# ydchen0806/CLC

Measured on AMD Instinct MI355X. Metric: images/sec fwd+bwd @256x256 bs8; bpp+PSNR parity vs ref, higher is better.
Workload: dtype f32; 1 GPU; CLC N=64 lambda=0.0067 MSE, 256x256 bs8/GPU, n_refs=1: fwd + RD loss + bwd + clip_grad_norm + AdamW + aux step (configs[1]); global_batch=8, parallelism=dp1, ranks_seen=1, collective=none, hip_graph=True

## Files before the change

clc_amd/csrc/conv_wino.hip:

```cpp
#include "common.h"

namespace {
#include "conv_common.h"

constexpr int TH = 8, TW = 16, HW = TW + 2, HPIX = (TH + 2) * HW;
constexpr int HALO_FLOATS = HPIX * 128;
constexpr int PIECES = HPIX / 2;

struct WinoParams {
  ConvParams c;
  const float* u;
  int items, ntn, ncg;
  unsigned u_bytes;
};

#ifndef WINO_AB
#define WINO_AB 0
#endif
#if WINO_AB & 32
__device__ unsigned long long wino_dbg[32];
#define WINO_STAMP(k) do { if (blockIdx.x == 0 && tid == 0 && it == i0 + 1) wino_dbg[k] = __builtin_amdgcn_s_memtime(); } while (0)
#else
#define WINO_STAMP(k) do { } while (0)
#endif
#define MFMA(a, b, c) __builtin_amdgcn_mfma_f32_32x32x2f32((a), (b), (c), 0, 0, 0)

constexpr int VB_FLOATS = 16 * 32 * 16;

template <bool SHUF>
__global__ __launch_bounds__(512, 1) void conv_wino_kernel(const WinoParams wp) {
  const ConvParams& p = wp.c;
  extern __shared__ __attribute__((aligned(16))) float smem[];
  float* halo = smem;
  float* bias_s = smem + HALO_FLOATS + 2 * VB_FLOATS;
  float* VV = smem + HALO_FLOATS;
  const int tid = threadIdx.x, lane = tid & 63, wave = tid >> 6;
  const int li = lane & 31, h = lane >> 5;
  const int tiles_w = p.W / TW, tiles_h = p.H / TH;
  const int KCT = wp.ncg * 4;
  const int NC16 = wp.ncg * 8;
  const int i0 = (int)((long)wp.items * blockIdx.x / gridDim.x), i1 = (int)((long)wp.items * (blockIdx.x + 1) / gridDim.x);
  const __amdgpu_buffer_rsrc_t xr = __builtin_amdgcn_make_buffer_rsrc(const_cast<float*>(p.x), 0, p.x_bytes, 0x00020000);
  const __amdgpu_buffer_rsrc_t ur = __builtin_amdgcn_make_buffer_rsrc(const_cast<float*>(wp.u), 0, wp.u_bytes, 0x00020000);
  const int q = tid & 3, t = (tid >> 2) & 31, part = tid >> 7;
  const int ty = t >> 3, tx = t & 7;
  const int wi = wave >> 1, nh = wave & 1;
  const int qo = tid & 15, to = tid >> 4;
  const int ra = part == 0 ? 0 : (part == 2 ? 2 : 1), rb = part == 0 ? 2 : (part == 1 ? 2 : (part == 2 ? 1 : 3));
  const float sg = part == 1 ? 1.f : -1.f;
  const int hbase = ((2 * ty + ra) * HW + 2 * tx) * 128, hdelta = (rb - ra) * HW * 128;
  const int sw0 = (tx & 3) << 2, sw1 = ((tx + 1) & 3) << 2;
  const int vdst = (part * 4 * 32 + t) * 16 + ((q ^ ((t >> 2) & 3)) << 2);
  int afo[2];
#pragma unroll
  for (int t8 = 0; t8 < 2; ++t8) afo[t8] = li * 16 + (((2 * t8 + h) ^ ((li >> 2) & 3)) << 2);
  const unsigned b_lane = (unsigned)lane * 16u;
  const bool lean = epilogue_is_lean(p);

  auto deposit = [&](int pt, int cg) {
    const int txx = pt % tiles_w, t2 = pt / tiles_w, tyy = t2 % tiles_h, n = t2 / tiles_h;
    const int oy0 = tyy * TH, ox0 = txx * TW;
    const int org = ((n * p.H + oy0 - 1) * p.W + ox0 - 1) * p.ldx + cg * 128;
    int hy = 0, hx = 2 * wave + h;
#pragma unroll 1
    for (int pc = wave; pc < PIECES; pc += 8) {
      const int iy = oy0 - 1 + hy, ix = ox0 - 1 + hx;
      const bool ok = (unsigned)iy < (unsigned)p.H && (unsigned)ix < (unsigned)p.W;
      const int c = li ^ (((hx >> 1) & 3) << 2);
      dma16(xr, halo + pc * 256, ok ? (unsigned)(org + (hy * p.W + hx) * p.ldx + c * 4) * 4u : kOOB);
      hx += 16;
      if (hx >= HW) { hx -= HW; ++hy; }
    }
  };

  int res_pt = -1, res_cg = -1;
  for (int it = i0; it < i1; ++it) {
    const int pt = it / wp.ntn, nt = it - pt * wp.ntn;
    const int txx = pt % tiles_w, t2 = pt / tiles_w, tyy = t2 % tiles_h, n = t2 / tiles_h;
    const int oy0 = tyy * TH, ox0 = txx * TW;
    f32x16 acc[4][2];
#pragma unroll
    for (int jj = 0; jj < 4; ++jj)
#pragma unroll
      for (int nbi = 0; nbi < 2; ++nbi)
#pragma unroll
        for (int r = 0; r < 16; ++r) acc[jj][nbi][r] = 0.f;
    f32x4 bq[2][2][2];
    auto load_b = [&](int slot, int jj, int c16) {
      const int kcg = c16 >> 1, t8g = 2 * (c16 & 1);
#pragma unroll
      for (int nbi = 0; nbi < 2; ++nbi) {
        const unsigned base = (unsigned)(((((nt * 16 + 4 * wi + jj) * KCT + kcg) * 4 + 2 * nh + nbi) * 4 + t8g)) * 1024u;
#pragma unroll
        for (int t8 = 0; t8 < 2; ++t8) bq[slot][nbi][t8] = buf_load4(ur, b_lane + base + (unsigned)(t8 * 1024));
      }
    };
    const float bias_v = (p.bias && tid < 128) ? p.bias[nt * 128 + tid] : 0.f;
    load_b(0, 0, 0);
    WINO_STAMP(0);

    for (int cg = 0; cg < wp.ncg; ++cg) {
      bool landed = cg == 0;
      if (pt != res_pt || cg != res_cg) {
        res_pt = pt; res_cg = cg;
        deposit(pt, cg);
        landed = false;
      }
      if (!landed) asm volatile("s_waitcnt vmcnt(0)" ::: "memory");
      __syncthreads();
      WINO_STAMP(1);
      if (cg == 0 && tid < 128) bias_s[tid] = bias_v;
      {
        f32x4 T[4];
#pragma unroll
        for (int c = 0; c < 4; ++c) {
          const float* src = halo + hbase + c * 128 + ((q ^ (c < 2 ? sw0 : sw1)) << 2);
          T[c] = *reinterpret_cast<const f32x4*>(src) + sg * *reinterpret_cast<const f32x4*>(src + hdelta);
        }
        float* dst = VV + vdst;
        *reinterpret_cast<f32x4*>(dst) = T[0] - T[2];
        *reinterpret_cast<f32x4*>(dst + 1 * 32 * 16) = T[1] + T[2];
        *reinterpret_cast<f32x4*>(dst + 2 * 32 * 16) = T[2] - T[1];
        *reinterpret_cast<f32x4*>(dst + 3 * 32 * 16) = T[1] - T[3];
      }
      WINO_STAMP(2);
#pragma unroll 1
      for (int kc = 0; kc < 8; ++kc) {
        __syncthreads();
        WINO_STAMP(3 + kc);
        const float* Vc = VV + (kc & 1) * VB_FLOATS;
        float* Vn = VV + ((kc + 1) & 1) * VB_FLOATS;
        const int c16 = cg * 8 + kc;
        f32x4 aq[2][2];
        f32x4 da[4], T[4];
#pragma unroll
        for (int t8 = 0; t8 < 2; ++t8) aq[0][t8] = *reinterpret_cast<const f32x4*>(Vc + (4 * wi) * 512 + afo[t8]);
        int npt = -1, ncg2 = 0;
        if (kc == 7) {
          npt = pt; ncg2 = cg + 1;
          if (ncg2 == wp.ncg) { ncg2 = 0; npt = it + 1 < i1 ? (it + 1) / wp.ntn : -1; }
          if (npt >= 0 && (npt != res_pt || ncg2 != res_cg)) { res_pt = npt; res_cg = ncg2; } else npt = -1;
          if (npt >= 0) deposit(npt, ncg2);
        }
#pragma unroll
        for (int g = 0; g < 4; ++g) {
          const int cur = g & 1;
          if (!(WINO_AB & 4)) {
            if (g < 3) load_b(cur ^ 1, g + 1, c16);
            else load_b(cur ^ 1, 0, c16 + 1 < NC16 ? c16 + 1 : 0);
          }
          if (g < 3) {
#pragma unroll
            for (int t8 = 0; t8 < 2; ++t8) aq[cur ^ 1][t8] = *reinterpret_cast<const f32x4*>(Vc + (4 * wi + g + 1) * 512 + afo[t8]);
          }
          if (WINO_AB & 8) {
          } else if (g == 0) {
            const int cb = (((kc + 1) & 7) * 4 + q);
#pragma unroll
            for (int c = 0; c < 4; ++c) da[c] = *reinterpret_cast<const f32x4*>(halo + hbase + c * 128 + ((cb ^ (c < 2 ? sw0 : sw1)) << 2));
          } else if (g == 1) {
            const int cb = (((kc + 1) & 7) * 4 + q);
#pragma unroll
            for (int c = 0; c < 4; ++c) {
              const f32x4 dbv = *reinterpret_cast<const f32x4*>(halo + hbase + hdelta + c * 128 + ((cb ^ (c < 2 ? sw0 : sw1)) << 2));
              T[c] = da[c] + sg * dbv;
            }
          } else if (g == 2) {
            float* dst = Vn + vdst;
            *reinterpret_cast<f32x4*>(dst) = T[0] - T[2];
            *reinterpret_cast<f32x4*>(dst + 1 * 32 * 16) = T[1] + T[2];
            *reinterpret_cast<f32x4*>(dst + 2 * 32 * 16) = T[2] - T[1];
            *reinterpret_cast<f32x4*>(dst + 3 * 32 * 16) = T[1] - T[3];
          }
          __builtin_amdgcn_sched_barrier(0);
#pragma unroll
          for (int t8 = 0; t8 < 2; ++t8)
#pragma unroll
            for (int ss = 0; ss < 4; ++ss)
#pragma unroll
              for (int nbi = 0; nbi < 2; ++nbi) {
                if (!(WINO_AB & 1)) acc[g][nbi] = MFMA(aq[cur][t8][ss], bq[cur][nbi][t8][ss], acc[g][nbi]);
                else acc[g][nbi][(t8 * 4 + ss) & 15] += aq[cur][t8][ss] * bq[cur][nbi][t8][ss];
              }
          __builtin_amdgcn_sched_barrier(0);
        }
      }
    }
    WINO_STAMP(11);
    asm volatile("s_waitcnt vmcnt(0)" ::: "memory");
    WINO_STAMP(12);
#pragma unroll 1
    for (int rd = 0; rd < ((WINO_AB & 2) ? 1 : 2); ++rd) {
      const int tyo = to >> 3, txo = to & 7;
      const int co = nt * 128 + ((qo >> 3) * 2 + rd) * 32 + (qo & 7) * 4;
      const f32x4 bv = *reinterpret_cast<const f32x4*>(bias_s + (co - nt * 128));
      __syncthreads();
      WINO_STAMP(13 + 3 * rd);
#pragma unroll
      for (int b = 0; b < 2; ++b) {
        float* dst = VV + ((wi * 2 + b) * 32) * 64;
#pragma unroll
        for (int r = 0; r < 16; ++r) {
          const float m0 = rd == 0 ? acc[0][0][r] : acc[0][1][r], m1 = rd == 0 ? acc[1][0][r] : acc[1][1][r];
          const float m2 = rd == 0 ? acc[2][0][r] : acc[2][1][r], m3 = rd == 0 ? acc[3][0][r] : acc[3][1][r];
          const float cv = b == 0 ? (m0 + m1) + m2 : (m1 - m2) - m3;
          const int row = (r & 3) + 8 * (r >> 2) + 4 * h;
          dst[row * 64 + ((nh * 32 + li) ^ (h << 5))] = cv;
        }
      }
      __syncthreads();
      WINO_STAMP(14 + 3 * rd);
      {
        const int col = (qo << 2) ^ (((to >> 2) & 1) << 5);
        f32x4 y[2][2];
#pragma unroll
        for (int b = 0; b < 2; ++b) {
          f32x4 c[4];
#pragma unroll
          for (int ii = 0; ii < 4; ++ii) c[ii] = *reinterpret_cast<const f32x4*>(VV + ((ii * 2 + b) * 32 + to) * 64 + col);
          y[0][b] = (c[0] + c[1]) + c[2];
          y[1][b] = (c[1] - c[2]) - c[3];
        }
        const int mrow0 = (n * p.OH + oy0 + 2 * tyo) * p.OW + ox0 + 2 * txo;
        if (lean) {
          if (!SHUF) {
#pragma unroll 1
            for (int a = 0; a < 2; ++a) {
              const size_t pix = (size_t)(mrow0 + a * p.OW);
              const f32x4 ya = a ? y[1][0] : y[0][0], yb = a ? y[1][1] : y[0][1];
              const Lean4In ia = lean_load4(p, pix, co), ib = lean_load4(p, pix + 1, co);
              lean_finish4(p, bv, ya, ia, pix, co);
              lean_finish4(p, bv, yb, ib, pix + 1, co);
            }
          } else {
#pragma unroll 1
            for (int a = 0; a < 2; ++a) {
              const f32x4 ya = a ? y[1][0] : y[0][0], yb = a ? y[1][1] : y[0][1];
              lean_store_shuffle4(p, bv, ya, n, oy0 + 2 * tyo + a, ox0 + 2 * txo, co);
              lean_store_shuffle4(p, bv, yb, n, oy0 + 2 * tyo + a, ox0 + 2 * txo + 1, co);
            }
          }
        } else if (!SHUF) {
#pragma unroll 1
          for (int a = 0; a < 2; ++a) {
            const size_t pix = (size_t)(mrow0 + a * p.OW);
            const f32x4 ya = a ? y[1][0] : y[0][0], yb = a ? y[1][1] : y[0][1];
            const Epi4In ia = epilogue_load4(p, pix, co), ib = epilogue_load4(p, pix + 1, co);
            epilogue_finish4(p, bv, ya, ia, pix, co);
            epilogue_finish4(p, bv, yb, ib, pix + 1, co);
          }
        } else {
#pragma unroll 1
          for (int a = 0; a < 2; ++a)
#pragma unroll 1
            for (int e = 0; e < 4; ++e) {
              epilogue_store(p, a ? y[1][0][e] : y[0][0][e], bv[e], mrow0 + a * p.OW, co + e, p.OH, p.OW, 0, 0);
              epilogue_store(p, a ? y[1][1][e] : y[0][1][e], bv[e], mrow0 + a * p.OW + 1, co + e, p.OH, p.OW, 0, 0);
            }
        }
      }
      WINO_STAMP(15 + 3 * rd);
    }
  }
}

constexpr int HALO2_FLOATS = HPIX * 64;
constexpr int V2_FLOATS = 16 * 32 * 16;
constexpr int PIECES2 = HPIX / 4;

template <bool SHUF>
__global__ __launch_bounds__(256, 2) void conv_wino64_kernel(const WinoParams wp) {
  const ConvParams& p = wp.c;
  extern __shared__ __attribute__((aligned(16))) float smem[];
  float* halo = smem;
  float* V = smem + HALO2_FLOATS;
  float* S = smem;
  const int tid = threadIdx.x, lane = tid & 63, wave = tid >> 6;
  const int li = lane & 31, h = lane >> 5;
  const int tiles_w = p.W / TW, tiles_h = p.H / TH;
  const int KCT = wp.ncg * 2;
  const int NC16 = wp.ncg * 4;
  const int i0 = (int)((long)wp.items * blockIdx.x / gridDim.x), i1 = (int)((long)wp.items * (blockIdx.x + 1) / gridDim.x);
  const __amdgpu_buffer_rsrc_t xr = __builtin_amdgcn_make_buffer_rsrc(const_cast<float*>(p.x), 0, p.x_bytes, 0x00020000);
  const __amdgpu_buffer_rsrc_t ur = __builtin_amdgcn_make_buffer_rsrc(const_cast<float*>(wp.u), 0, wp.u_bytes, 0x00020000);
  const int q = tid & 3, t = (tid >> 2) & 31, half = tid >> 7;
  const int ty = t >> 3, tx = t & 7;
  const int qo = tid & 15;
  const bool lean = epilogue_is_lean(p);
  int afo[2];
#pragma unroll
  for (int t8 = 0; t8 < 2; ++t8) afo[t8] = li * 16 + (((2 * t8 + h) ^ ((li >> 2) & 3)) << 2);
  const unsigned b_lane = (unsigned)lane * 16u;

  int cur_pt = -1, cur_cg = -1;
  for (int it = i0; it < i1; ++it) {
    const int pt = it / wp.ntn, nt = it - pt * wp.ntn;
    const int txx = pt % tiles_w, t2 = pt / tiles_w, tyy = t2 % tiles_h, n = t2 / tiles_h;
    const int oy0 = tyy * TH, ox0 = txx * TW;
    f32x16 acc[4][2];
#pragma unroll
    for (int s = 0; s < 4; ++s)
#pragma unroll
      for (int nb = 0; nb < 2; ++nb)
#pragma unroll
        for (int r = 0; r < 16; ++r) acc[s][nb][r] = 0.f;
    f32x4 bq[2][2][2];
    auto load_b = [&](int slot, int s, int c16) {
      const int kcg = c16 >> 1, t8g = 2 * (c16 & 1);
#pragma unroll
      for (int nb = 0; nb < 2; ++nb) {
        const unsigned base = (unsigned)((((((nt >> 1) * 16 + 4 * wave + s) * KCT + kcg) * 4 + 2 * (nt & 1) + nb) * 4 + t8g)) * 1024u;
#pragma unroll
        for (int t8 = 0; t8 < 2; ++t8) bq[slot][nb][t8] = buf_load4(ur, b_lane + base + (unsigned)(t8 * 1024));
      }
    };
    load_b(0, 0, 0);

    for (int cg = 0; cg < wp.ncg; ++cg) {
      if (pt != cur_pt || cg != cur_cg) {
        cur_pt = pt; cur_cg = cg;
        const int org = ((n * p.H + oy0 - 1) * p.W + ox0 - 1) * p.ldx + cg * 64;
        int hy = 0, hx = 4 * wave + (lane >> 4);
#pragma unroll 1
        for (int pc = wave; pc < PIECES2; pc += 4) {
          const int iy = oy0 - 1 + hy, ix = ox0 - 1 + hx;
          const bool ok = (unsigned)iy < (unsigned)p.H && (unsigned)ix < (unsigned)p.W;
          const int c = (lane & 15) ^ (((hx >> 1) & 3) << 2);
          dma16(xr, halo + pc * 256, ok ? (unsigned)(org + (hy * p.W + hx) * p.ldx + c * 4) * 4u : kOOB);
          hx += 16;
          if (hx >= HW) { hx -= HW; ++hy; }
        }
        asm volatile("s_waitcnt vmcnt(0)" ::: "memory");
      }
#pragma unroll 1
      for (int kc = 0; kc < 4; ++kc) {
        __syncthreads();
        {
          const int cidx = kc * 4 + q;
          f32x4 d[3][4];
#pragma unroll
          for (int r = 0; r < 3; ++r)
#pragma unroll
            for (int c = 0; c < 4; ++c) {
              const int hy = 2 * ty + r + half, hx = 2 * tx + c;
              d[r][c] = *reinterpret_cast<const f32x4*>(halo + (hy * HW + hx) * 64 + ((cidx ^ (((hx >> 1) & 3) << 2)) << 2));
            }
          f32x4 T[2][4];
#pragma unroll
          for (int c = 0; c < 4; ++c) {
            if (half == 0) { T[0][c] = d[0][c] - d[2][c]; T[1][c] = d[1][c] + d[2][c]; }
            else           { T[0][c] = d[1][c] - d[0][c]; T[1][c] = d[0][c] - d[2][c]; }
          }
#pragma unroll
          for (int i = 0; i < 2; ++i) {
            const f32x4 v0 = T[i][0] - T[i][2], v1 = T[i][1] + T[i][2], v2 = T[i][2] - T[i][1], v3 = T[i][1] - T[i][3];
            float* dst = V + (((2 * half + i) * 4) * 32 + t) * 16 + ((q ^ ((t >> 2) & 3)) << 2);
            *reinterpret_cast<f32x4*>(dst) = v0;
            *reinterpret_cast<f32x4*>(dst + 1 * 32 * 16) = v1;
            *reinterpret_cast<f32x4*>(dst + 2 * 32 * 16) = v2;
            *reinterpret_cast<f32x4*>(dst + 3 * 32 * 16) = v3;
          }
        }
        __syncthreads();
        const int c16 = cg * 4 + kc;
        f32x4 aq[2][2];
#pragma unroll
        for (int t8 = 0; t8 < 2; ++t8) aq[0][t8] = *reinterpret_cast<const f32x4*>(V + (4 * wave) * 512 + afo[t8]);
#pragma unroll
        for (int s = 0; s < 4; ++s) {
          const int cur = s & 1;
          if (s < 3) {
            load_b(cur ^ 1, s + 1, c16);
#pragma unroll
            for (int t8 = 0; t8 < 2; ++t8) aq[cur ^ 1][t8] = *reinterpret_cast<const f32x4*>(V + (4 * wave + s + 1) * 512 + afo[t8]);
          } else {
            load_b(cur ^ 1, 0, c16 + 1 < NC16 ? c16 + 1 : 0);
          }
          __builtin_amdgcn_sched_barrier(0);
#pragma unroll
          for (int t8 = 0; t8 < 2; ++t8)
#pragma unroll
            for (int ss = 0; ss < 4; ++ss)
#pragma unroll
              for (int nb = 0; nb < 2; ++nb) acc[s][nb] = MFMA(aq[cur][t8][ss], bq[cur][nb][t8][ss], acc[s][nb]);
          __builtin_amdgcn_sched_barrier(0);
        }
      }
    }
    cur_pt = -1;
    {
      const int co = nt * 64 + (qo >> 3) * 32 + (qo & 7) * 4;
      const f32x4 bv = epilogue_bias4(p.bias, co);
      __syncthreads();
#pragma unroll
      for (int b = 0; b < 2; ++b) {
        float* dst = S + ((wave * 2 + b) * 32) * 64;
#pragma unroll
        for (int nb = 0; nb < 2; ++nb)
#pragma unroll
          for (int r = 0; r < 16; ++r) {
            const float cv = b == 0 ? (acc[0][nb][r] + acc[1][nb][r]) + acc[2][nb][r] : (acc[1][nb][r] - acc[2][nb][r]) - acc[3][nb][r];
            const int row = (r & 3) + 8 * (r >> 2) + 4 * h;
            dst[row * 64 + ((nb * 32 + li) ^ (h << 5))] = cv;
          }
      }
      __syncthreads();
#pragma unroll 1
      for (int tt = 0; tt < 2; ++tt) {
        const int to = (tid >> 4) + 16 * tt, tyo = to >> 3, txo = to & 7;
        const int col = (qo << 2) ^ (((to >> 2) & 1) << 5);
        f32x4 y[2][2];
#pragma unroll
        for (int b = 0; b < 2; ++b) {
          f32x4 c[4];
#pragma unroll
          for (int ii = 0; ii < 4; ++ii) c[ii] = *reinterpret_cast<const f32x4*>(S + ((ii * 2 + b) * 32 + to) * 64 + col);
          y[0][b] = (c[0] + c[1]) + c[2];
          y[1][b] = (c[1] - c[2]) - c[3];
        }
        const int mrow0 = (n * p.OH + oy0 + 2 * tyo) * p.OW + ox0 + 2 * txo;
#pragma unroll 1
        for (int a = 0; a < 2; ++a) {
          const size_t pix = (size_t)(mrow0 + a * p.OW);
          const f32x4 ya = a ? y[1][0] : y[0][0], yb = a ? y[1][1] : y[0][1];
          if (lean) {
            if (!SHUF) {
              const Lean4In ia = lean_load4(p, pix, co), ib = lean_load4(p, pix + 1, co);
              lean_finish4(p, bv, ya, ia, pix, co);
              lean_finish4(p, bv, yb, ib, pix + 1, co);
            } else {
              lean_store_shuffle4(p, bv, ya, n, oy0 + 2 * tyo + a, ox0 + 2 * txo, co);
              lean_store_shuffle4(p, bv, yb, n, oy0 + 2 * tyo + a, ox0 + 2 * txo + 1, co);
            }
          } else if (!SHUF) {
            const Epi4In ia = epilogue_load4(p, pix, co), ib = epilogue_load4(p, pix + 1, co);
            epilogue_finish4(p, bv, ya, ia, pix, co);
            epilogue_finish4(p, bv, yb, ib, pix + 1, co);
          } else {
#pragma unroll 1
            for (int e = 0; e < 4; ++e) {
              epilogue_store(p, ya[e], bv[e], (int)pix, co + e, p.OH, p.OW, 0, 0);
              epilogue_store(p, yb[e], bv[e], (int)pix + 1, co + e, p.OH, p.OW, 0, 0);
            }
          }
        }
      }
    }
    __syncthreads();
  }
}

__device__ __forceinline__ void wino_u_one(const float* __restrict__ w, float* __restrict__ out, long e, int K, int flip) {
  const int kq = (int)(e % (K / 4)), n = (int)(e / (K / 4)), k = kq * 4;
  f32x4 g[3][3];
#pragma unroll
  for (int a = 0; a < 3; ++a)
#pragma unroll
    for (int b = 0; b < 3; ++b) {
      const int tap = flip ? 8 - (a * 3 + b) : a * 3 + b;
      g[a][b] = *reinterpret_cast<const f32x4*>(w + ((size_t)n * 9 + tap) * K + k);
    }
  f32x4 tt[4][3];
#pragma unroll
  for (int b = 0; b < 3; ++b) {
    tt[0][b] = g[0][b];
    tt[1][b] = 0.5f * ((g[0][b] + g[1][b]) + g[2][b]);
    tt[2][b] = 0.5f * ((g[0][b] - g[1][b]) + g[2][b]);
    tt[3][b] = g[2][b];
  }
  const int KCT = K / 32, nt = n >> 7, nb = (n & 127) >> 5, kcg = k >> 5, kk = k & 31, t8 = kk >> 3, hh = (kk & 7) >> 2;
  const int lane = (n & 31) + 32 * hh;
#pragma unroll
  for (int i = 0; i < 4; ++i) {
    f32x4 u[4];
    u[0] = tt[i][0];
    u[1] = 0.5f * ((tt[i][0] + tt[i][1]) + tt[i][2]);
    u[2] = 0.5f * ((tt[i][0] - tt[i][1]) + tt[i][2]);
    u[3] = tt[i][2];
#pragma unroll
    for (int j = 0; j < 4; ++j) {
      const size_t idx = ((((((size_t)nt * 16 + (i * 4 + j)) * KCT + kcg) * 4 + nb) * 4 + t8) * 64 + lane);
      *reinterpret_cast<f32x4*>(out + idx * 4) = u[j];
    }
  }
}
__global__ void filter_wino_kernel(const float* __restrict__ w, float* __restrict__ out, int N, int K, int flip) {
  const long e = (long)blockIdx.x * blockDim.x + threadIdx.x;
  if (e >= (long)N * K / 4) return;
  wino_u_one(w, out, e, K, flip);
}
__global__ void filter_wino_batched_kernel(const clc_wino_entry* __restrict__ table, int n_entries) {
  int lo = 0, hi = n_entries - 1;
  const int b = blockIdx.x;
  while (lo < hi) {
    const int mid = (lo + hi + 1) >> 1;
    if (table[mid].block_begin <= b) lo = mid; else hi = mid - 1;
  }
  const clc_wino_entry en = table[lo];
  const long e = (long)(b - en.block_begin) * blockDim.x + threadIdx.x;
  if (e >= (long)en.N * en.K / 4) return;
  wino_u_one(en.w, en.out, e, en.K, en.flip);
}

}

extern "C" int clc_filter_wino(const float* w, float* out, int N, int K, int flip, clc_stream_t stream) {
  CLC_CHECK(w && out && N > 0 && N % 64 == 0 && K > 0 && K % 64 == 0 && aligned16(w) && aligned16(out),
            "clc_filter_wino: rows and channels must be positive multiples of 64, pointers 16-B aligned (got N=%d K=%d)", N, K);
  const long total = (long)N * K / 4;
  hipLaunchKernelGGL(filter_wino_kernel, dim3((unsigned)((total + 255) / 256)), dim3(256), 0, (hipStream_t)stream, w, out, N, K, flip);
  CLC_LAUNCH_CHECK();
  return 0;
}
extern "C" int clc_filter_wino_batched(const clc_wino_entry* table_dev, int n_entries, int total_blocks, clc_stream_t stream) {
  CLC_CHECK(table_dev && n_entries > 0 && total_blocks > 0, "clc_filter_wino_batched: bad args");
  hipLaunchKernelGGL(filter_wino_batched_kernel, dim3(total_blocks), dim3(256), 0, (hipStream_t)stream, table_dev, n_entries);
  CLC_LAUNCH_CHECK();
  return 0;
}

int clc_conv_wino_launch(const void* conv_params, const float* u, hipStream_t st) {
  const ConvParams& p = *reinterpret_cast<const ConvParams*>(conv_params);
  if (!u || p.ks != 3 || p.stride != 1 || p.pad != 1 || p.Cin % 64 || p.Cin > 1024 || p.Cout % 64 || p.H % TH || p.W % TW || p.OH != p.H || p.OW != p.W) return 0;
  if (p.xs || p.in_op != CLC_IN_NONE || p.group_rows || p.bf16 || p.ksplit > 1 || p.ldx % 4 || !aligned16(p.x) || !aligned16(u)) return 0;
  const bool shuf = p.shuffle != 0;
  if (!shuf && !p.vec_epi) return 0;
  const size_t ub = (size_t)((p.Cout + 127) / 128 * 128) * 16 * p.Cin * 4;
  if (ub >= (1ull << 31)) return 0;
  const int mode = clc_tuning[CLC_TUNE_WINO];
  const int ptiles = p.N * (p.H / TH) * (p.W / TW);
  const bool can128 = p.Cin % 128 == 0 && p.Cout % 128 == 0 && !(mode & 8);
  const bool wide = can128 && ptiles * (p.Cout / 128) >= 192;
  if (!wide && (!(mode & 4) || ptiles * (p.Cout / 64) < 128)) return 0;
  const int nw = wide ? 128 : 64;
  WinoParams wp;
  wp.c = p;
  wp.u = u;
  wp.ntn = p.Cout / nw;
  wp.ncg = p.Cin / nw;
  wp.items = ptiles * wp.ntn;
  wp.u_bytes = (unsigned)ub;
  static PerDeviceOnce once[2];
  const int k = shuf ? 1 : 0;
  if (wide) {
    const int grid = wp.items < 256 ? wp.items : 256;
    const int lds = (HALO_FLOATS + 2 * VB_FLOATS + 128) * 4;
    static PerDeviceOnce oncep[2];
    if (shuf) {
      if (oncep[0].first()) (void)hipFuncSetAttribute(reinterpret_cast<const void*>(conv_wino_kernel<true>), hipFuncAttributeMaxDynamicSharedMemorySize, lds);
      hipLaunchKernelGGL(conv_wino_kernel<true>, dim3(grid), dim3(512), lds, st, wp);
    } else {
      if (oncep[1].first()) (void)hipFuncSetAttribute(reinterpret_cast<const void*>(conv_wino_kernel<false>), hipFuncAttributeMaxDynamicSharedMemorySize, lds);
      hipLaunchKernelGGL(conv_wino_kernel<false>, dim3(grid), dim3(512), lds, st, wp);
    }
  } else {
    const int grid = wp.items < 512 ? wp.items : 512;
    const int lds = (HALO2_FLOATS + V2_FLOATS) * 4;
    if (shuf) {
      if (once[k].first()) (void)hipFuncSetAttribute(reinterpret_cast<const void*>(conv_wino64_kernel<true>), hipFuncAttributeMaxDynamicSharedMemorySize, lds);
      hipLaunchKernelGGL(conv_wino64_kernel<true>, dim3(grid), dim3(256), lds, st, wp);
    } else {
      if (once[k].first()) (void)hipFuncSetAttribute(reinterpret_cast<const void*>(conv_wino64_kernel<false>), hipFuncAttributeMaxDynamicSharedMemorySize, lds);
      hipLaunchKernelGGL(conv_wino64_kernel<false>, dim3(grid), dim3(256), lds, st, wp);
    }
  }
  CLC_LAUNCH_CHECK();
  return (13 << 20) | ((wide ? 0 : 1) << 12) | (wp.ncg << 4) | ((p.transposed ? 1 : 0) << 1) | (shuf ? 1 : 0);
}

#if WINO_AB & 32
extern "C" int clc_wino_debug(unsigned long long* out_host) {
  return (int)hipMemcpyFromSymbol(out_host, HIP_SYMBOL(wino_dbg), sizeof(unsigned long long) * 32);
}
#endif
```

Before: 340.7 images/sec.

## Compute Winograd input transform in registers and interleave with MFMA in wino64 kernel

The 64-channel Winograd conv kernel no longer writes the transformed input tile V to LDS and reads it back. Each wave now builds its own transform rows directly from the halo into MFMA A-operand registers, using a per-wave sign FMA, and interleaves those halo reads and transform steps with the MFMA blocks and weight buffer loads. This removes two barriers and the LDS round trip per k-chunk, shrinks the LDS footprint to the output staging buffer, and batches the lean epilogue's loads ahead of its stores. The cost is more registers and redundant halo reads across waves, with inline asm pinning the adds.

```diff
diff --git a/clc_amd/csrc/conv_wino.hip b/clc_amd/csrc/conv_wino.hip
--- a/clc_amd/csrc/conv_wino.hip
+++ b/clc_amd/csrc/conv_wino.hip
@@ -265,17 +265,21 @@
 }
 
 constexpr int HALO2_FLOATS = HPIX * 64;
-constexpr int V2_FLOATS = 16 * 32 * 16;
+constexpr int S2_FLOATS = 16 * 32 * 32;
 constexpr int PIECES2 = HPIX / 4;
+static_assert(HALO2_FLOATS <= S2_FLOATS, "the halo lies inside the output round's image");
+__device__ __forceinline__ int wino64_swz(int hy, int hx) { return ((hx >> 1) & 3) | (((hy >> 1) & 3) << 2); }
+__device__ __forceinline__ float add1(float a, float b) { float r; asm("v_add_f32 %0, %1, %2" : "=v"(r) : "v"(a), "v"(b)); return r; }
+__device__ __forceinline__ float sub1(float a, float b) { float r; asm("v_sub_f32 %0, %1, %2" : "=v"(r) : "v"(a), "v"(b)); return r; }
+__device__ __forceinline__ float fma1(float s, float b, float a) { float r; asm("v_fma_f32 %0, %1, %2, %3" : "=v"(r) : "s"(s), "v"(b), "v"(a)); return r; }
 
 template <bool SHUF>
 __global__ __launch_bounds__(256, 2) void conv_wino64_kernel(const WinoParams wp) {
   const ConvParams& p = wp.c;
   extern __shared__ __attribute__((aligned(16))) float smem[];
   float* halo = smem;
-  float* V = smem + HALO2_FLOATS;
   float* S = smem;
-  const int tid = threadIdx.x, lane = tid & 63, wave = tid >> 6;
+  const int tid = threadIdx.x, lane = tid & 63, wave = __builtin_amdgcn_readfirstlane(tid >> 6);
   const int li = lane & 31, h = lane >> 5;
   const int tiles_w = p.W / TW, tiles_h = p.H / TH;
   const int KCT = wp.ncg * 2;
@@ -283,16 +287,26 @@
   const int i0 = (int)((long)wp.items * blockIdx.x / gridDim.x), i1 = (int)((long)wp.items * (blockIdx.x + 1) / gridDim.x);
   const __amdgpu_buffer_rsrc_t xr = __builtin_amdgcn_make_buffer_rsrc(const_cast<float*>(p.x), 0, p.x_bytes, 0x00020000);
   const __amdgpu_buffer_rsrc_t ur = __builtin_amdgcn_make_buffer_rsrc(const_cast<float*>(wp.u), 0, wp.u_bytes, 0x00020000);
-  const int q = tid & 3, t = (tid >> 2) & 31, half = tid >> 7;
-  const int ty = t >> 3, tx = t & 7;
+  const int ty = li >> 3, tx = li & 7;
   const int qo = tid & 15;
   const bool lean = epilogue_is_lean(p);
-  int afo[2];
-#pragma unroll
-  for (int t8 = 0; t8 < 2; ++t8) afo[t8] = li * 16 + (((2 * t8 + h) ^ ((li >> 2) & 3)) << 2);
+  const int ra = wave == 0 ? 0 : (wave == 2 ? 2 : 1), rb = wave == 0 ? 2 : (wave == 1 ? 2 : (wave == 2 ? 1 : 3));
+  const float sg = wave == 1 ? 1.f : -1.f;
+  int pa[2][2];
+#pragma unroll
+  for (int rr = 0; rr < 2; ++rr)
+#pragma unroll
+    for (int ch = 0; ch < 2; ++ch) {
+      const int hy = 2 * ty + (rr ? rb : ra);
+      pa[rr][ch] = (hy * HW + 2 * tx) * 256 + ((h ^ wino64_swz(hy, 2 * tx + 2 * ch)) << 4);
+    }
+  const char* hb = reinterpret_cast<const char*>(halo);
+  auto read_row = [&](f32x4 (&d)[4], int rr, int kx) {
+#pragma unroll
+    for (int c = 0; c < 4; ++c) d[c] = *reinterpret_cast<const f32x4*>(hb + ((pa[rr][c >> 1] ^ kx) + c * 256));
+  };
   const unsigned b_lane = (unsigned)lane * 16u;
 
-  int cur_pt = -1, cur_cg = -1;
   for (int it = i0; it < i1; ++it) {
     const int pt = it / wp.ntn, nt = it - pt * wp.ntn;
     const int txx = pt % tiles_w, t2 = pt / tiles_w, tyy = t2 % tiles_h, n = t2 / tiles_h;
@@ -304,94 +318,88 @@
       for (int nb = 0; nb < 2; ++nb)
 #pragma unroll
         for (int r = 0; r < 16; ++r) acc[s][nb][r] = 0.f;
-    f32x4 bq[2][2][2];
-    auto load_b = [&](int slot, int s, int c16) {
-      const int kcg = c16 >> 1, t8g = 2 * (c16 & 1);
-#pragma unroll
-      for (int nb = 0; nb < 2; ++nb) {
-        const unsigned base = (unsigned)((((((nt >> 1) * 16 + 4 * wave + s) * KCT + kcg) * 4 + 2 * (nt & 1) + nb) * 4 + t8g)) * 1024u;
-#pragma unroll
-        for (int t8 = 0; t8 < 2; ++t8) bq[slot][nb][t8] = buf_load4(ur, b_lane + base + (unsigned)(t8 * 1024));
-      }
+    f32x4 bq[4][2];
+    auto load_b = [&](int s, int c16, int t8) {
+      const int kcg = c16 >> 1, t8g = 2 * (c16 & 1) + t8;
+#pragma unroll
+      for (int nb = 0; nb < 2; ++nb)
+        bq[s][nb] = buf_load4(ur, b_lane + (unsigned)((((((nt >> 1) * 16 + 4 * wave + s) * KCT + kcg) * 4 + 2 * (nt & 1) + nb) * 4 + t8g)) * 1024u);
     };
-    load_b(0, 0, 0);
+#pragma unroll
+    for (int s = 0; s < 4; ++s) load_b(s, 0, 0);
+    WINO_STAMP(0);
 
     for (int cg = 0; cg < wp.ncg; ++cg) {
-      if (pt != cur_pt || cg != cur_cg) {
-        cur_pt = pt; cur_cg = cg;
+      if (cg) __syncthreads();
+      {
         const int org = ((n * p.H + oy0 - 1) * p.W + ox0 - 1) * p.ldx + cg * 64;
         int hy = 0, hx = 4 * wave + (lane >> 4);
 #pragma unroll 1
         for (int pc = wave; pc < PIECES2; pc += 4) {
           const int iy = oy0 - 1 + hy, ix = ox0 - 1 + hx;
           const bool ok = (unsigned)iy < (unsigned)p.H && (unsigned)ix < (unsigned)p.W;
-          const int c = (lane & 15) ^ (((hx >> 1) & 3) << 2);
+          const int c = (lane & 15) ^ wino64_swz(hy, hx);
           dma16(xr, halo + pc * 256, ok ? (unsigned)(org + (hy * p.W + hx) * p.ldx + c * 4) * 4u : kOOB);
           hx += 16;
           if (hx >= HW) { hx -= HW; ++hy; }
         }
         asm volatile("s_waitcnt vmcnt(0)" ::: "memory");
       }
+      __syncthreads();
+      WINO_STAMP(1);
+      f32x4 aq[2][4];
+      f32x4 da[4], db[4];
+      auto rows_T = [&]() {
+#pragma unroll
+        for (int c = 0; c < 4; ++c)
+#pragma unroll
+          for (int e = 0; e < 4; ++e) da[c][e] = fma1(sg, db[c][e], da[c][e]);
+      };
+      auto cols_B = [&](f32x4 (&v)[4]) {
+#pragma unroll
+        for (int e = 0; e < 4; ++e) {
+          v[0][e] = sub1(da[0][e], da[2][e]);
+          v[1][e] = add1(da[1][e], da[2][e]);
+          v[2][e] = sub1(da[2][e], da[1][e]);
+          v[3][e] = sub1(da[1][e], da[3][e]);
+        }
+      };
+      read_row(da, 0, 0);
+      read_row(db, 1, 0);
+      rows_T();
+      cols_B(aq[0]);
+      WINO_STAMP(2);
 #pragma unroll 1
       for (int kc = 0; kc < 4; ++kc) {
-        __syncthreads();
-        {
-          const int cidx = kc * 4 + q;
-          f32x4 d[3][4];
-#pragma unroll
-          for (int r = 0; r < 3; ++r)
-#pragma unroll
-            for (int c = 0; c < 4; ++c) {
-              const int hy = 2 * ty + r + half, hx = 2 * tx + c;
-              d[r][c] = *reinterpret_cast<const f32x4*>(halo + (hy * HW + hx) * 64 + ((cidx ^ (((hx >> 1) & 3) << 2)) << 2));
-            }
-          f32x4 T[2][4];
-#pragma unroll
-          for (int c = 0; c < 4; ++c) {
-            if (half == 0) { T[0][c] = d[0][c] - d[2][c]; T[1][c] = d[1][c] + d[2][c]; }
-            else           { T[0][c] = d[1][c] - d[0][c]; T[1][c] = d[0][c] - d[2][c]; }
-          }
-#pragma unroll
-          for (int i = 0; i < 2; ++i) {
-            const f32x4 v0 = T[i][0] - T[i][2], v1 = T[i][1] + T[i][2], v2 = T[i][2] - T[i][1], v3 = T[i][1] - T[i][3];
-            float* dst = V + (((2 * half + i) * 4) * 32 + t) * 16 + ((q ^ ((t >> 2) & 3)) << 2);
-            *reinterpret_cast<f32x4*>(dst) = v0;
-            *reinterpret_cast<f32x4*>(dst + 1 * 32 * 16) = v1;
-            *reinterpret_cast<f32x4*>(dst + 2 * 32 * 16) = v2;
-            *reinterpret_cast<f32x4*>(dst + 3 * 32 * 16) = v3;
-          }
-        }
-        __syncthreads();
+        if (cg == 0) WINO_STAMP(3 + kc);
         const int c16 = cg * 4 + kc;
-        f32x4 aq[2][2];
-#pragma unroll
-        for (int t8 = 0; t8 < 2; ++t8) aq[0][t8] = *reinterpret_cast<const f32x4*>(V + (4 * wave) * 512 + afo[t8]);
-#pragma unroll
-        for (int s = 0; s < 4; ++s) {
-          const int cur = s & 1;
-          if (s < 3) {
-            load_b(cur ^ 1, s + 1, c16);
-#pragma unroll
-            for (int t8 = 0; t8 < 2; ++t8) aq[cur ^ 1][t8] = *reinterpret_cast<const f32x4*>(V + (4 * wave + s + 1) * 512 + afo[t8]);
-          } else {
-            load_b(cur ^ 1, 0, c16 + 1 < NC16 ? c16 + 1 : 0);
-          }
-          __builtin_amdgcn_sched_barrier(0);
-#pragma unroll
-          for (int t8 = 0; t8 < 2; ++t8)
+#pragma unroll
+        for (int t8 = 0; t8 < 2; ++t8) {
+          const int kxn = t8 == 0 ? (4 * kc + 2) << 4 : (4 * ((kc + 1) & 3)) << 4;
+          const int c16n = t8 == 0 ? c16 : (c16 + 1 < NC16 ? c16 + 1 : 0);
+#pragma unroll
+          for (int s = 0; s < 4; ++s) {
+            if (s == 0) read_row(da, 0, kxn);
+            else if (s == 1) read_row(db, 1, kxn);
+            else if (s == 2) rows_T();
+            else cols_B(aq[t8 ^ 1]);
+            __builtin_amdgcn_sched_barrier(0);
 #pragma unroll
             for (int ss = 0; ss < 4; ++ss)
 #pragma unroll
-              for (int nb = 0; nb < 2; ++nb) acc[s][nb] = MFMA(aq[cur][t8][ss], bq[cur][nb][t8][ss], acc[s][nb]);
-          __builtin_amdgcn_sched_barrier(0);
-        }
-      }
-    }
-    cur_pt = -1;
+              for (int nb = 0; nb < 2; ++nb) acc[s][nb] = MFMA(aq[t8][s][ss], bq[s][nb][ss], acc[s][nb]);
+            load_b(s, c16n, t8 ^ 1);
+            __builtin_amdgcn_sched_barrier(0);
+          }
+        }
+      }
+    }
+    WINO_STAMP(11);
     {
       const int co = nt * 64 + (qo >> 3) * 32 + (qo & 7) * 4;
       const f32x4 bv = epilogue_bias4(p.bias, co);
       __syncthreads();
+      WINO_STAMP(13);
 #pragma unroll
       for (int b = 0; b < 2; ++b) {
         float* dst = S + ((wave * 2 + b) * 32) * 64;
@@ -405,11 +413,9 @@
           }
       }
       __syncthreads();
-#pragma unroll 1
-      for (int tt = 0; tt < 2; ++tt) {
-        const int to = (tid >> 4) + 16 * tt, tyo = to >> 3, txo = to & 7;
+      WINO_STAMP(14);
+      auto read_y = [&](int to, f32x4 (&y)[2][2]) {
         const int col = (qo << 2) ^ (((to >> 2) & 1) << 5);
-        f32x4 y[2][2];
 #pragma unroll
         for (int b = 0; b < 2; ++b) {
           f32x4 c[4];
@@ -418,34 +424,60 @@
           y[0][b] = (c[0] + c[1]) + c[2];
           y[1][b] = (c[1] - c[2]) - c[3];
         }
-        const int mrow0 = (n * p.OH + oy0 + 2 * tyo) * p.OW + ox0 + 2 * txo;
-#pragma unroll 1
-        for (int a = 0; a < 2; ++a) {
-          const size_t pix = (size_t)(mrow0 + a * p.OW);
-          const f32x4 ya = a ? y[1][0] : y[0][0], yb = a ? y[1][1] : y[0][1];
-          if (lean) {
-            if (!SHUF) {
-              const Lean4In ia = lean_load4(p, pix, co), ib = lean_load4(p, pix + 1, co);
-              lean_finish4(p, bv, ya, ia, pix, co);
-              lean_finish4(p, bv, yb, ib, pix + 1, co);
-            } else {
+      };
+      if (lean && !SHUF) {
+        f32x4 y[2][2][2];
+        Lean4In in[2][2][2];
+        size_t px[2][2];
+#pragma unroll
+        for (int tt = 0; tt < 2; ++tt) {
+          const int to = (tid >> 4) + 16 * tt, tyo = to >> 3, txo = to & 7;
+          read_y(to, y[tt]);
+#pragma unroll
+          for (int a = 0; a < 2; ++a) px[tt][a] = (size_t)((n * p.OH + oy0 + 2 * tyo + a) * p.OW + ox0 + 2 * txo);
+        }
+#pragma unroll
+        for (int tt = 0; tt < 2; ++tt)
+#pragma unroll
+          for (int a = 0; a < 2; ++a)
+#pragma unroll
+            for (int b = 0; b < 2; ++b) in[tt][a][b] = lean_load4(p, px[tt][a] + b, co);
+#pragma unroll
+        for (int tt = 0; tt < 2; ++tt)
+#pragma unroll
+          for (int a = 0; a < 2; ++a)
+#pragma unroll
+            for (int b = 0; b < 2; ++b) lean_finish4(p, bv, y[tt][a][b], in[tt][a][b], px[tt][a] + b, co);
+      } else {
+#pragma unroll 1
+        for (int tt = 0; tt < 2; ++tt) {
+          const int to = (tid >> 4) + 16 * tt, tyo = to >> 3, txo = to & 7;
+          f32x4 y[2][2];
+          read_y(to, y);
+          const int mrow0 = (n * p.OH + oy0 + 2 * tyo) * p.OW + ox0 + 2 * txo;
+#pragma unroll 1
+          for (int a = 0; a < 2; ++a) {
+            const size_t pix = (size_t)(mrow0 + a * p.OW);
+            const f32x4 ya = a ? y[1][0] : y[0][0], yb = a ? y[1][1] : y[0][1];
+            if (lean) {
               lean_store_shuffle4(p, bv, ya, n, oy0 + 2 * tyo + a, ox0 + 2 * txo, co);
               lean_store_shuffle4(p, bv, yb, n, oy0 + 2 * tyo + a, ox0 + 2 * txo + 1, co);
+            } else if (!SHUF) {
+              const Epi4In ia = epilogue_load4(p, pix, co), ib = epilogue_load4(p, pix + 1, co);
+              epilogue_finish4(p, bv, ya, ia, pix, co);
+              epilogue_finish4(p, bv, yb, ib, pix + 1, co);
+            } else {
+#pragma unroll 1
+              for (int e = 0; e < 4; ++e) {
+                epilogue_store(p, ya[e], bv[e], (int)pix, co + e, p.OH, p.OW, 0, 0);
+                epilogue_store(p, yb[e], bv[e], (int)pix + 1, co + e, p.OH, p.OW, 0, 0);
+              }
             }
-          } else if (!SHUF) {
-            const Epi4In ia = epilogue_load4(p, pix, co), ib = epilogue_load4(p, pix + 1, co);
-            epilogue_finish4(p, bv, ya, ia, pix, co);
-            epilogue_finish4(p, bv, yb, ib, pix + 1, co);
-          } else {
-#pragma unroll 1
-            for (int e = 0; e < 4; ++e) {
-              epilogue_store(p, ya[e], bv[e], (int)pix, co + e, p.OH, p.OW, 0, 0);
-              epilogue_store(p, yb[e], bv[e], (int)pix + 1, co + e, p.OH, p.OW, 0, 0);
-            }
-          }
-        }
-      }
-    }
+          }
+        }
+      }
+    }
+    WINO_STAMP(15);
     __syncthreads();
   }
 }
@@ -555,7 +587,7 @@
     }
   } else {
     const int grid = wp.items < 512 ? wp.items : 512;
-    const int lds = (HALO2_FLOATS + V2_FLOATS) * 4;
+    const int lds = S2_FLOATS * 4;
     if (shuf) {
       if (once[k].first()) (void)hipFuncSetAttribute(reinterpret_cast<const void*>(conv_wino64_kernel<true>), hipFuncAttributeMaxDynamicSharedMemorySize, lds);
       hipLaunchKernelGGL(conv_wino64_kernel<true>, dim3(grid), dim3(256), lds, st, wp);
```

Result: faster. 344.6 images/sec (median of 6 runs) (+1.2%).
